# floatingtrees/video-VAE

Measured on AMD Instinct MI355X. Metric: video frames/sec (fwd+bwd) at Bx3x16x256x256, higher is better.
Workload: dtype bf16; 1 GPU; C3: full VideoVAE (enc 9 / dec 12 FactoredAttention + 3D-conv UNet) train step, B=4/GPU x 3x16x256x256, bf16 compute, fp32 params, recon+KL loss, clip+Adam; flavour=model, params=170631304, global_batch=4, frames_per_clip=16, parallelism=dp1, launch_mode=hipgraph(fwd+bwd) + eager all-reduce/clip/Adam

## Files before the change

### include/vvae_hip.h

```cpp
#ifndef VVAE_HIP_H
#define VVAE_HIP_H
#include <stddef.h>
#include <stdint.h>

#ifdef __cplusplus
extern "C" {
#endif

#define VVAE_DT_F32 0
#define VVAE_DT_BF16 1
#define VVAE_ERR_BAD_ARG 1001
#define VVAE_ERR_WORKSPACE 1002
#define VVAE_ERR_LIBRARY 1003

size_t vvae_conv3d_workspace_bytes(int N, int T, int H, int W, int Cin, int Cout, int kt, int kh, int kw, int dtype,
                                   int which );
int vvae_conv3d_fwd(const void* x, int ldx, const float* w, const float* bias, void* y, int ldy,
                    int N, int T, int H, int W, int Cin, int Cout, int kt, int kh, int kw, int dtype,
                    void* ws, size_t ws_bytes, void* stream);
int vvae_conv3d_dgrad(const void* dy, int lddy, const float* w, void* dx, int lddx,
                      int N, int T, int H, int W, int Cin, int Cout, int kt, int kh, int kw, int dtype,
                      void* ws, size_t ws_bytes, void* stream);
int vvae_conv3d_wgrad(const void* x, int ldx, const void* dy, int lddy, float* dw, float* dbias,
                      int N, int T, int H, int W, int Cin, int Cout, int kt, int kh, int kw, int dtype,
// ... 205 lines not shown
                          const float* sin_table, float* part, int A, int S, int heads, int D, float eps, int dtype, void* stream);

int vvae_layernorm_supported(int C, int dtype);
int vvae_layernorm_bwd_blocks(long rows, int C, int dtype);
int vvae_delay_us(int us, void* stream);
int vvae_layernorm_fwd_config(int fwd_cap);
int vvae_gn_config(int stream_blocks);
int vvae_layernorm_config(int bwd_cap);
int vvae_layernorm_fwd_mode(int late_stage);
int vvae_layernorm_fwd(const void* x, void* y, const float* gamma, const float* beta, float* mean, float* rstd,
                       const void* addend, void* xsum, long rows, int C, int inner, long outer_pitch, long inner_pitch, float eps,
                       int dtype, void* stream);
int vvae_layernorm_bwd(const void* x, const void* dy, const float* gamma, const float* mean, const float* rstd, const void* dres,
                       void* dx, float* part, long rows, int C, int inner, long outer_pitch, long inner_pitch, int dtype,
                       void* stream);

size_t vvae_loss_part_floats(int B, long M);
int vvae_reparam_kl_fwd(const void* mean, const void* logvar, const float* eps, const float* mask, float* z, float* kl,
                        float* part, int B, int T, long per, int dtype, void* stream);
int vvae_reparam_kl_bwd(const void* mean, const void* logvar, const float* eps, const float* mask, const float* dz,
                        const float* gkl, void* dmean, void* dlogvar, int B, int T, long per, int dtype, void* stream);

int vvae_masked_mse_mae_fwd(const void* video, const void* recon, const float* mask, float* mse, float* mae,
                            float* part, int B, int T, long P, int video_div, int dtype, void* stream);
int vvae_masked_mse_mae_bwd(const void* video, const void* recon, const float* mask, const float* gmse, const float* gmae,
                            void* drecon, int B, int T, long P, int video_div, int dtype, void* stream);

int vvae_gemm_tn_supported(int M, int N, int K, int lda, int ldb);
size_t vvae_gemm_tn_ws_bytes(int M, int N, int K);
int vvae_gemm_tn_bf16(const void* A, int lda, const void* B, int ldb, float* C, float* db, int M, int N, int K,
                      void* ws, size_t ws_bytes, void* stream);
int vvae_gemm_tn_grouped_bf16(const void* const* A, const int* lda, const void* const* B, const int* ldb, float* const* C,
                              float* const* db, const int* M, const int* N, int n, int K, void* stream);
int vvae_gemm_tn_use_big_tiles(int on);

int vvae_sqnorm_blocks(long n);
int vvae_sqnorm_partials(const float* g, long n, double* part, void* stream);
int vvae_adam_clip_step(float* p, const float* g, float* m, float* v, void* p_bf16, long n, const double* gnorm_part, int nparts,
                        double* gnorm_sq_out, float gscale, float max_norm, float lr, float b1, float b2, float eps, long count,
                        void* stream);
int vvae_cast_f32_to_bf16(const float* x, void* y, long n, void* stream);
int vvae_gemm_nt_supported(int M, int N, int K, int lda, int ldb, int ldc);
int vvae_gemm_nt_bf16(const void* A, int lda, const void* B, int ldb, void* C, int ldc, const float* bias, const void* res,
                      int ldr, void* C2, int ldc2, int epi, int M, int N, int K, void* stream);
int vvae_gemm_pp_supported(int M, int N, int K, int lda, int ldb, int ldc);
int vvae_gemm_pp_bf16(const void* A, int lda, const void* B, int ldb, void* C, int ldc, const float* bias, const void* res,
                      int ldr, void* C2, int ldc2, int epi, int M, int N, int K, void* stream);
int vvae_gemm_pp_ablate(int bits);
int vvae_gemm_pp_final_ring(int on);
int vvae_gemm_nt_stagger(int units);
int vvae_gemm_nt_persistent(int on);
int vvae_gemm_nt_prefetch(int dist);
int vvae_gemm_nt_prefetch_mask(int mask);

int vvae_sum_rows(const float* part, int rows, int cols, float* out, void* stream);
int vvae_fold_rows_grouped(const void* const* part, float* const* d0, float* const* d1, const int* rows, const int* cols,
                           const int* n0, int n, void* stream);
int vvae_copy_grouped(const float* const* src, float* const* dst, const long* count, int n, void* stream);

int vvae_selftest_xor_lane(const float* x, float* y, double* yd, int n, int o, void* stream);

#ifdef __cplusplus
}
#endif
#endif
```

### video_vae_amd/csrc/gemm_tn256.hip

```cpp
#include "common.hpp"

#ifndef TN_ABL
#define TN_ABL 0
#endif

namespace tn256 {

#ifdef TN_STAMPS
__device__ unsigned long long g_tn_stamps[256 * 4];
#endif

typedef __bf16 bf16x8 __attribute__((ext_vector_type(8)));
typedef short s16x4v __attribute__((ext_vector_type(4)));

constexpr int BM = 256, BN = 256, KS = 32, S = 4;
constexpr int ROW = 512;
constexpr int OPB = KS * ROW;
constexpr int STAGE = 2 * OPB;
constexpr int LDS_BYTES = S * STAGE;
constexpr int P = 4;
#ifndef TN_ALATE
#define TN_ALATE 3
#endif
constexpr int ALATE = TN_ALATE;

struct Dims { int M, N, K, lda, ldb, klen, tiles_m, tiles_n; };

template <int N> __device__ __forceinline__ void wait_vm()
{
    static_assert(N >= 0 && N < 64, "vmcnt is 6 bits");
    __builtin_amdgcn_s_waitcnt((N & 15) | ((N >> 4) << 14) | 0x0F70);
}

__device__ __forceinline__ void glds16(const void* g, unsigned char* lds_wave_base)
{
    __builtin_amdgcn_global_load_lds((const __attribute__((address_space(1))) void*)g,
                                     (__attribute__((address_space(3))) void*)lds_wave_base, 16, 0, 0);
}

__device__ __forceinline__ void tn256_tile(const bf16_t* __restrict__ A, const bf16_t* __restrict__ B, int lda, int ldb, int m0, int n0, int k_beg,
                                             int nk, float* __restrict__ out, int ld_out, float* __restrict__ out_db)
{
    extern __shared__ __attribute__((aligned(16))) unsigned char smem[];
    const int tid = threadIdx.x, lane = tid & 63, wave = tid >> 6;
    const int wm = wave >> 2, wn = wave & 3, grp = wave >> 2;

    const bf16_t* ga[2];
    const bf16_t* gb[2];
#pragma unroll
    for (int i = 0; i < 2; ++i) {
        const int row = 2 * (2 * wave + i) + (lane >> 5);
        const int chunk = (lane & 31) ^ ((row & 7) << 1);
        ga[i] = A + (long)(k_beg + row) * lda + m0 + chunk * 8;
        gb[i] = B + (long)(k_beg + row) * ldb + n0 + chunk * 8;
    }
    auto issue = [&](int t, int stage) {
        if ((TN_ABL & 1) && t >= S) return;
        unsigned char* sb = smem + stage * STAGE + (2 * wave) * 1024;
        const long ka = (long)t * KS * lda, kb = (long)t * KS * ldb;
        glds16(ga[0] + ka, sb);
        glds16(ga[1] + ka, sb + 1024);
        glds16(gb[0] + kb, sb + OPB);
        glds16(gb[1] + kb, sb + OPB + 1024);
    };
    auto wait_tiles = [&](int tiles_in_flight) {
        if (tiles_in_flight >= 2) wait_vm<2 * P>(); else if (tiles_in_flight == 1) wait_vm<P>(); else wait_vm<0>();
    };

    const int g4 = lane >> 4, q4 = (lane >> 2) & 3, p4 = lane & 3;
    const int r1 = 4 * g4 + q4, sw = (r1 & 7) << 1;
    int aoff[8], boff[4];
#pragma unroll
    for (int ib = 0; ib < 8; ++ib) aoff[ib] = r1 * ROW + ((((8 * wm + ib) * 2 + (p4 >> 1)) ^ sw) << 4) + (p4 & 1) * 8;
#pragma unroll
// ... 68 lines not shown
                    __builtin_amdgcn_sched_group_barrier(0x008, 2, 0);
                } else {
                    __builtin_amdgcn_sched_group_barrier(0x008, 4, 0);
                }
            }
        }
        if (do_bias && !(TN_ABL & 4)) {
#pragma unroll
            for (int jb = 0; jb < 4; ++jb) accb[jb] = __builtin_amdgcn_mfma_f32_16x16x32_bf16(ones, bfr[jb], accb[jb], 0, 0, 0);
        }
        asm volatile("s_waitcnt lgkmcnt(0)" ::: "memory");
        vvae_phase_barrier();
        st = st + 1 == S ? 0 : st + 1;
    }
    if (!grp) vvae_phase_barrier();
#ifdef TN_STAMPS
    if (tid == 0 && blockIdx.x < 256) { g_tn_stamps[blockIdx.x * 4 + 2] = __builtin_amdgcn_s_memtime(); g_tn_stamps[blockIdx.x * 4 + 3] = __builtin_amdgcn_s_memrealtime(); }
#endif

    const int nl = lane & 15;
#pragma unroll
    for (int ib = 0; ib < 8; ++ib)
#pragma unroll
        for (int jb = 0; jb < 4; ++jb)
#pragma unroll
            for (int j = 0; j < 4; ++j) {
                const int m = m0 + 128 * wm + 16 * ib + 4 * g4 + j;
                out[(long)m * ld_out + n0 + 64 * wn + 16 * jb + nl] = acc[ib][jb][j];
            }
    if (do_bias && g4 == 0) {
#pragma unroll
        for (int jb = 0; jb < 4; ++jb) out_db[n0 + 64 * wn + 16 * jb + nl] = accb[jb][0];
    }
}

__global__ __launch_bounds__(512, 1) void gemm_tn256_kernel(const bf16_t* __restrict__ A, const bf16_t* __restrict__ B, float* __restrict__ slab,
                                                            float* __restrict__ slab_db, Dims d)
{
    const int nwg = gridDim.x, q8 = nwg >> 3, r8 = nwg & 7, xcd = blockIdx.x & 7;
    const int L = (xcd < r8 ? xcd * (q8 + 1) : r8 * (q8 + 1) + (xcd - r8) * q8) + (blockIdx.x >> 3);
    const int tiles = d.tiles_m * d.tiles_n;
    const int sp = L / tiles, tile = L - sp * tiles;
    const int tm = tile / d.tiles_n, tn = tile - tm * d.tiles_n;
    const int k_beg = sp * d.klen;
    int k_end = k_beg + d.klen;
    if (k_end > d.K) k_end = d.K;
    tn256_tile(A, B, d.lda, d.ldb, tm * BM, tn * BN, k_beg, (k_end - k_beg) / KS, slab + (long)sp * d.M * d.N, d.N,
               (slab_db && tm == 0) ? slab_db + (long)sp * d.N : nullptr);
}

struct GroupProb { const bf16_t* A; const bf16_t* B; float* C; float* db; int M, N, lda, ldb, tiles_m, tiles_n, tile_start; };
constexpr int GROUP_MAX = 64;
struct GroupArgs { GroupProb p[GROUP_MAX]; int nprob, K; };

__global__ __launch_bounds__(512, 1) void gemm_tn256_grouped_kernel(GroupArgs g)
{
    const int nwg = gridDim.x, q8 = nwg >> 3, r8 = nwg & 7, xcd = blockIdx.x & 7;
    const int L = (xcd < r8 ? xcd * (q8 + 1) : r8 * (q8 + 1) + (xcd - r8) * q8) + (blockIdx.x >> 3);
    int pi = 0;
    for (int i = 1; i < g.nprob; ++i) pi = L >= g.p[i].tile_start ? i : pi;
    const GroupProb& P = g.p[pi];
    const int tile = L - P.tile_start;
    int tm, tn;
    if (P.tiles_m <= P.tiles_n) { tn = tile / P.tiles_m; tm = tile - tn * P.tiles_m; }
    else { tm = tile / P.tiles_n; tn = tile - tm * P.tiles_n; }
    tn256_tile(P.A, P.B, P.lda, P.ldb, tm * BM, tn * BN, 0, g.K / KS, P.C, P.N, (P.db && tm == 0) ? P.db : nullptr);
}

int pick_splits(int M, int N, int K)
{
    const int tiles = (M / BM) * (N / BN);
    int s = 256 / tiles;
    const int max_s = K / (8 * KS);
    if (s > max_s) s = max_s;
    if (s < 1) s = 1;
    return s;
}

bool supported(int M, int N, int K, int lda, int ldb)
{
    return M > 0 && N > 0 && K > 0 && M % BM == 0 && N % BN == 0 && K % KS == 0 && lda % 8 == 0 && ldb % 8 == 0 && lda >= M && ldb >= N;
}

int launch(const void* A, int lda, const void* B, int ldb, float* slab, float* slab_db, int M, int N, int K, int splits, int* used,
           hipStream_t s)
{
    int klen = (K + splits - 1) / splits;
    klen = (klen + KS - 1) / KS * KS;
    *used = (K + klen - 1) / klen;
    Dims d{M, N, K, lda, ldb, klen, M / BM, N / BN};
    static bool attr_done = false;
    if (!attr_done) {
        hipError_t e = hipFuncSetAttribute((const void*)gemm_tn256_kernel, hipFuncAttributeMaxDynamicSharedMemorySize, LDS_BYTES);
        if (e != hipSuccess) return (int)e;
        attr_done = true;
    }
    hipLaunchKernelGGL(gemm_tn256_kernel, dim3(d.tiles_m * d.tiles_n * *used), dim3(512), LDS_BYTES, s, (const bf16_t*)A, (const bf16_t*)B,
                       slab, slab_db, d);
    hipError_t e = hipGetLastError();
    return e == hipSuccess ? 0 : (int)e;
}

int launch_grouped(const GroupArgs& g, int total_tiles, hipStream_t s)
{
    static bool attr_done = false;
    if (!attr_done) {
        hipError_t e = hipFuncSetAttribute((const void*)gemm_tn256_grouped_kernel, hipFuncAttributeMaxDynamicSharedMemorySize, LDS_BYTES);
        if (e != hipSuccess) return (int)e;
        attr_done = true;
    }
    hipLaunchKernelGGL(gemm_tn256_grouped_kernel, dim3(total_tiles), dim3(512), LDS_BYTES, s, g);
    hipError_t e = hipGetLastError();
    return e == hipSuccess ? 0 : (int)e;
}

}

#ifdef TN_STAMPS
extern "C" int vvae_gemm_tn_stamps(unsigned long long* host_out)
{
    return (int)hipMemcpyFromSymbol(host_out, HIP_SYMBOL(tn256::g_tn_stamps), sizeof(unsigned long long) * 256 * 4, 0, hipMemcpyDeviceToHost);
}
#endif

extern "C" int vvae_gemm_tn_grouped_bf16(const void* const* A, const int* lda, const void* const* B, const int* ldb, float* const* C,
                                         float* const* db, const int* M, const int* N, int n, int K, void* stream)
{
    if (!A || !lda || !B || !ldb || !C || !db || !M || !N || n <= 0 || n > tn256::GROUP_MAX || K <= 0 || K % tn256::KS) return VVAE_ERR_BAD_ARG;
    tn256::GroupArgs g;
    g.nprob = n; g.K = K;
    int tiles = 0;
    for (int i = 0; i < n; ++i) {
        if (!A[i] || !B[i] || !C[i] || !tn256::supported(M[i], N[i], K, lda[i], ldb[i]) || ((uintptr_t)A[i] % 16) || ((uintptr_t)B[i] % 16) ||
            ((uintptr_t)C[i] % 16)) return VVAE_ERR_BAD_ARG;
        g.p[i] = tn256::GroupProb{(const bf16_t*)A[i], (const bf16_t*)B[i], C[i], db[i], M[i], N[i], lda[i], ldb[i], M[i] / tn256::BM,
                                  N[i] / tn256::BN, tiles};
        tiles += (M[i] / tn256::BM) * (N[i] / tn256::BN);
    }
    return tn256::launch_grouped(g, tiles, (hipStream_t)stream);
}
```

### video_vae_amd/csrc/loss_optim.hip

```cpp
#include "common.hpp"

namespace {

__device__ __forceinline__ float block_sum(float v, float* red) {
    v = wave_sum(v);
    const int lane = threadIdx.x & 63, wave = threadIdx.x >> 6;
    if (lane == 0) red[wave] = v;
    __syncthreads();
    float t = 0.f;
    if (threadIdx.x == 0) for (int i = 0; i < (int)(blockDim.x >> 6); ++i) t += red[i];
    __syncthreads();
    return t;
}

__device__ __forceinline__ float seq_len(const float* __restrict__ mrow, int T) {
    float s = 0.f;
    for (int t = 0; t < T; ++t) s += mrow[t];
    return fmaxf(s, 1.0f);
}

template <typename T_>
__global__ __launch_bounds__(256) void reparam_kl_fwd_kernel(const T_* __restrict__ mean, const T_* __restrict__ logvar,
                                                             const float* __restrict__ eps, const float* __restrict__ mask,
                                                             float* __restrict__ z, float* __restrict__ kl_part, int T, long per,
// ... 280 lines not shown
__global__ __launch_bounds__(256) void adam_clip_kernel(float* __restrict__ p, const float* __restrict__ g, float* __restrict__ m,
                                                        float* __restrict__ v, bf16_t* __restrict__ p_bf16, long n,
                                                        const double* __restrict__ gnorm_part, int nparts,
                                                        double* __restrict__ gnorm_sq_out, float gscale, float max_norm, float lr,
                                                        float b1, float b2, float eps, float c1, float c2)
{
    float clip = gscale;
    if (gnorm_part) {
        __shared__ double dred[256];
        double a = 0.0;
        for (int i = threadIdx.x; i < nparts; i += 256) a += gnorm_part[i];
        dred[threadIdx.x] = a;
        __syncthreads();
        for (int st = 128; st > 0; st >>= 1) {
            if ((int)threadIdx.x < st) dred[threadIdx.x] += dred[threadIdx.x + st];
            __syncthreads();
        }
        const double tot = dred[0];
        if (gnorm_sq_out && blockIdx.x == 0 && threadIdx.x == 0) *gnorm_sq_out = tot;
        const float gn = gscale * (float)sqrt(tot);
        if (gn >= max_norm) clip = gscale * max_norm / gn;
    }
    for (long i = (long)blockIdx.x * 256 + threadIdx.x; i < n; i += (long)gridDim.x * 256) {
        const float gi = g[i] * clip;
        const float mi = b1 * m[i] + (1.f - b1) * gi;
        const float vi = b2 * v[i] + (1.f - b2) * gi * gi;
        m[i] = mi; v[i] = vi;
        const float pi = p[i] - lr * (mi / c1) / (sqrtf(vi / c2) + eps);
        p[i] = pi;
        if (p_bf16) p_bf16[i] = f2bf(pi);
    }
}

__global__ __launch_bounds__(256) void cast_f32_bf16_kernel(const float* __restrict__ x, bf16_t* __restrict__ y, long n)
{
    for (long i = (long)blockIdx.x * 256 + threadIdx.x; i < n; i += (long)gridDim.x * 256) y[i] = f2bf(x[i]);
}

inline int pick_epb(long M, int B) {
    long want = 2048 / (B > 0 ? B : 1); if (want < 1) want = 1;
    long epb = (M + want - 1) / want;
    epb = ((epb + 2047) / 2048) * 2048;
    return (int)epb;
}

}

extern "C" size_t vvae_loss_part_floats(int B, long M)
{
    if (B <= 0 || M <= 0) return 0;
    return (size_t)2 * B * ceil_div(M, (long)pick_epb(M, B));
}

extern "C" int vvae_reparam_kl_fwd(const void* mean, const void* logvar, const float* eps, const float* mask, float* z, float* kl,
                                   float* part, int B, int T, long per, int dtype, void* stream)
{
    if (!mean || !logvar || (!z && !kl) || (z && !eps) || (kl && !part) || B <= 0 || T <= 0 || per <= 0) return VVAE_ERR_BAD_ARG;
    hipStream_t s = (hipStream_t)stream;
    const long M = (long)T * per;
    const int epb = pick_epb(M, B);
    dim3 grid(ceil_div(M, epb), B);
    float* klp = kl ? part : nullptr;
    if (dtype == VVAE_DT_F32)
        hipLaunchKernelGGL((reparam_kl_fwd_kernel<float>), grid, dim3(256), 0, s, (const float*)mean, (const float*)logvar, eps, mask, z, klp, T, per, epb);
    else if (dtype == VVAE_DT_BF16)
        hipLaunchKernelGGL((reparam_kl_fwd_kernel<bf16_t>), grid, dim3(256), 0, s, (const bf16_t*)mean, (const bf16_t*)logvar, eps, mask, z, klp, T, per, epb);
// ... 85 lines not shown
    } else return VVAE_ERR_BAD_ARG;
    VVAE_LAUNCH_CHECK();
    return 0;
}

extern "C" int vvae_sqnorm_blocks(long n)
{
    if (n <= 0) return 0;
    long blocks = n / 1024 + 1; if (blocks > SQN_MAX_BLOCKS) blocks = SQN_MAX_BLOCKS;
    return (int)blocks;
}

extern "C" int vvae_sqnorm_partials(const float* g, long n, double* part, void* stream)
{
    if (!g || !part || n <= 0 || ((uintptr_t)g % 16) != 0) return VVAE_ERR_BAD_ARG;
    hipLaunchKernelGGL(sqnorm_kernel, dim3((unsigned)vvae_sqnorm_blocks(n)), dim3(256), 0, (hipStream_t)stream, g, n, part);
    VVAE_LAUNCH_CHECK();
    return 0;
}

extern "C" int vvae_adam_clip_step(float* p, const float* g, float* m, float* v, void* p_bf16, long n, const double* gnorm_part,
                                   int nparts, double* gnorm_sq_out, float gscale, float max_norm, float lr, float b1, float b2,
                                   float eps, long count, void* stream)
{
    if (!p || !g || !m || !v || n <= 0 || count < 1 || (gnorm_part && (nparts <= 0 || nparts > SQN_MAX_BLOCKS))) return VVAE_ERR_BAD_ARG;
    const float c1 = 1.f - powf(b1, (float)count), c2 = 1.f - powf(b2, (float)count);
    long blocks = n / 1024 + 1; if (blocks > 4096) blocks = 4096;
    hipLaunchKernelGGL(adam_clip_kernel, dim3((unsigned)blocks), dim3(256), 0, (hipStream_t)stream, p, g, m, v, (bf16_t*)p_bf16, n,
                       gnorm_part, nparts, gnorm_sq_out, gscale, max_norm, lr, b1, b2, eps, c1, c2);
    VVAE_LAUNCH_CHECK();
    return 0;
}

extern "C" int vvae_cast_f32_to_bf16(const float* x, void* y, long n, void* stream)
{
    if (!x || !y || n <= 0) return VVAE_ERR_BAD_ARG;
    long blocks = n / 1024 + 1; if (blocks > 4096) blocks = 4096;
    hipLaunchKernelGGL(cast_f32_bf16_kernel, dim3((unsigned)blocks), dim3(256), 0, (hipStream_t)stream, x, (bf16_t*)y, n);
    VVAE_LAUNCH_CHECK();
    return 0;
}

namespace {
__global__ __launch_bounds__(256) void sum_rows_kernel(const float* __restrict__ part, int rows, int cols, float* __restrict__ out)
{
    __shared__ float4 red[32][8];
    const int cq = threadIdx.x & 7, rl = threadIdx.x >> 3;
    const int c = (blockIdx.x * 8 + cq) * 4;
    float4 s = make_float4(0.f, 0.f, 0.f, 0.f);
    if (c < cols) {
        for (int r0 = rl; r0 < rows; r0 += 32 * 16) {
            float4 v[16];
#pragma unroll
            for (int i = 0; i < 16; ++i) {
                const int r = r0 + 32 * i;
                v[i] = r < rows ? *reinterpret_cast<const float4*>(part + (long)r * cols + c) : make_float4(0.f, 0.f, 0.f, 0.f);
            }
#pragma unroll
            for (int i = 0; i < 16; ++i) { s.x += v[i].x; s.y += v[i].y; s.z += v[i].z; s.w += v[i].w; }
        }
    }
    red[rl][cq] = s;
    __syncthreads();
    for (int st = 16; st > 0; st >>= 1) {
        if (rl < st) {
            const float4 a = red[rl][cq], b = red[rl + st][cq];
// ... 251 lines not shown
```

### video_vae_amd/graph.py

```python
import ctypes
import gc

import torch

from . import loss as L
from . import ops


_NODE_TYPES = {0: "kernel", 1: "memcpy", 2: "memset", 3: "host", 4: "graph", 5: "empty", 6: "wait_event", 7: "event_record"}
_HIP = [None]


def graph_node_census(graph):
    raw = getattr(graph, "raw_cuda_graph", None)
    if raw is None:
        return None
    try:
        handle = raw()
        if _HIP[0] is None:
            _HIP[0] = ctypes.CDLL("libamdhip64.so")
        hip = _HIP[0]
        n = ctypes.c_size_t(0)
        if hip.hipGraphGetNodes(ctypes.c_void_p(handle), None, ctypes.byref(n)) != 0:
            return None
# ... 48 lines not shown
        self.graph = None
        self.debug_dot = debug_dot
        self._capture(warmup)

    @staticmethod
    def _unit(loss):
        return ops.unit_grad(loss) if (loss.dtype == torch.float32 and loss.dim() == 0) else None

    def _loss(self):
        emask = L.compact_mask(self.mask)
        if self.rl:
            return L.loss_fn(self.model, self.video, emask, self.mask, self.rngs, self.hparams, self.ploss, self.vgg_params)
        return L.loss_fn_plain(self.model, self.video, emask, self.mask, self.rngs, self.hparams)

    @staticmethod
    def _tensors(out):
        outs = out if isinstance(out, (tuple, list)) else (out,)
        return [o for o in outs if isinstance(o, torch.Tensor) and o.requires_grad]

    def _stage0(self):
        grabbed = {}
        hooks = [m.register_forward_hook(lambda mod, inp, out, j=j: grabbed.setdefault(j, []).append(out)) for j, m in enumerate(self.cut_modules)]
        try:
            loss, aux = self._loss()
        finally:
            for h in hooks:
                h.remove()
        self._cuts = []
        for j in range(len(self.cut_modules)):
            if len(grabbed.get(j, [])) != 1 or not self._tensors(grabbed[j][0]):
                raise RuntimeError("split capture expects every cut block of the encoder to run once and hand on differentiable tensors")
            self._cuts.append(self._tensors(grabbed[j][0]))
        opt = self.opt
        opt.external = set()
        opt.hooks_active = False
        params = [opt.params[i] for i in self.stage_idx[0]]
        with ops.deferred_wgrad(opt):
            grads = torch.autograd.grad(loss, params + self._cuts[0], grad_outputs=self._unit(loss), allow_unused=True)
        self._gcut = list(grads[len(params):])
        opt.land_subset(self.stage_idx[0], grads[:len(params)])
        return loss.detach(), {k: v.detach() for k, v in aux.items() if k != "reconstruction"}

    def _stage(self, st):
        opt = self.opt
        pairs = [(c, g) for c, g in zip(self._cuts[st - 1], self._gcut) if g is not None]
        params = [opt.params[i] for i in self.stage_idx[st]]
        nxt = self._cuts[st] if st < len(self._cuts) else []
        with ops.deferred_wgrad(opt):
            grads = torch.autograd.grad([c for c, _ in pairs], params + nxt, grad_outputs=[g for _, g in pairs], allow_unused=True)
        self._gcut = list(grads[len(params):])
        opt.land_subset(self.stage_idx[st], grads[:len(params)])
        if st == self.nstages - 1:
            opt.landed = [True] * len(opt.buckets)
            self._cuts = self._gcut = None

    def _prelaunch(self, st):
        opt = self.opt
        if opt.reducer is not None and opt.defer_reduce:
            if st == 0:
                opt.reducer.reset()
            for b, bs in enumerate(self.bucket_stage):
                if bs == st:
                    opt.reducer.launch(b)
                    opt.prelaunched.add(b)

    def _pass(self):
        if not self.split:
            return self._fwd_bwd()
        out = self._stage0()
        for st in range(1, self.nstages):
            self._prelaunch(st - 1)
            self._stage(st)
        return out

    def _fwd_bwd(self):
        loss, aux = self._loss()
        self.opt.external = set()
        self.opt.hooks_active = False
        with ops.deferred_wgrad(self.opt):
            grads = torch.autograd.grad(loss, self.opt.params, grad_outputs=self._unit(loss), allow_unused=True)
        self.opt.land_all(grads)
        return loss.detach(), {k: v.detach() for k, v in aux.items() if k != "reconstruction"}

    def _check_one_stream(self):
        from .optim import STREAM_TAG, accumulate_grad_node
        from ._lib import VvaeError
        if not self.video.is_cuda:
            return
        want = self.stream.cuda_stream
        with torch.cuda.stream(self.stream):
            for name, prm in zip(self.opt.names, self.opt.params):
                node = accumulate_grad_node(prm)
                have = node.metadata.get(STREAM_TAG) if node is not None else None
                if have is not None and have != want:
                    raise VvaeError(
                        f"GraphedTrainStep: parameter {name!r} has already taken part in an eager backward on stream {have:#x} and that pass's "
                        f"autograd graph is still alive, but the capture would run on stream {want:#x}.  One stream for the whole run: build the "
                        "model, run the eager steps and capture on the same non-default stream (pass it as stream=..., as train.py does), or drop "
                        "every tensor of the eager passes (loss, aux) before capturing.")

    def _refill(self):
        for name, (kind, buf) in self.noise.items():
            buf.normal_(generator=self.gen) if kind == "normal" else buf.uniform_(generator=self.gen)

    def _capture(self, warmup):
        opt = self.opt
        self.stream = self.capture_stream if self.capture_stream is not None else torch.cuda.Stream()
        self.stream.wait_stream(torch.cuda.current_stream())
        if getattr(self.model, "_kl", None) is not None:
            self.model._kl = None
# ... 22 lines not shown
            opt.zero_grad()
        torch.cuda.synchronize()
        gc.collect()
        try:
            g = torch.cuda.CUDAGraph(keep_graph=True)
        except TypeError:
            g = torch.cuda.CUDAGraph()
        if self.debug_dot:
            g.enable_debug_mode()
        mode = "thread_local" if opt.reducer is not None else "global"
        if self.split:
            with torch.cuda.graph(g, stream=self.stream, capture_error_mode=mode):
                self.loss, self.aux = self._stage0()
            for st in range(1, self.nstages):
                try:
                    gs = torch.cuda.CUDAGraph(keep_graph=True)
                except TypeError:
                    gs = torch.cuda.CUDAGraph()
                with torch.cuda.graph(gs, stream=self.stream, pool=g.pool(), capture_error_mode=mode):
                    self._stage(st)
                self.graphs.append(gs)
        else:
            with torch.cuda.graph(g, stream=self.stream, capture_error_mode=mode):
                self.loss, self.aux = self._fwd_bwd()
        if not all(opt.landed):
            raise RuntimeError("a gradient bucket did not land inside the captured backward (parameter without gradient)")
        self.census = [graph_node_census(x) for x in [g] + self.graphs]
        for c in self.census:
            if c and c.get("memset", 0):
                raise RuntimeError(f"the captured train step holds {c['memset']} hipGraph memset node(s) ({c}): on ROCm 7.2 a replayed memset node writes "
                                   "garbage, and whatever it was meant to zero (e.g. the semaphore of a multi-block framework reduction) misbehaves on "
                                   "replay.  Replace the op that issued hipMemsetAsync (DESIGN.md section 3, tools/memset_node_probe.py).")
        self.graph = g
        if self.debug_dot:
            g.debug_dump(self.debug_dot)
        opt.update()
        with torch.no_grad():
            opt.p.copy_(snap[0]); opt.m.copy_(snap[1]); opt.v.copy_(snap[2])
        opt.count = snap[3]
        opt.refresh_shadow()

    def __call__(self, video=None, mask=None, noise=None):
        if video is not None:
            self.video.copy_(video)
        if mask is not None:
            self.mask.copy_(mask)
        if noise is None:
            self._refill()
        else:
            if set(noise) != set(self.noise):
                raise KeyError(f"noise for {sorted(noise)} given, the captured step draws {sorted(self.noise)}")
            for name, t in noise.items():
                self.noise[name][1].copy_(t)
        self.graph.replay()
        for st, gs in enumerate(self.graphs, start=1):
            self._prelaunch(st - 1)
            gs.replay()
        self.opt.update()
        return self.loss, self.aux
```

### video_vae_amd/ops.py

```python
import ctypes
import os
import sys

import torch
import torch.nn.functional as F

from ._lib import lib, check, VvaeError

DT = {torch.float32: 0, torch.bfloat16: 1}

_NOTED = set()


def note_fallback(key, message):
    if key in _NOTED:
        return
    _NOTED.add(key)
    import os
    import sys
    if os.environ.get("RANK", "0") == "0":
        print(f"[video_vae_amd] fallback: {message}", file=sys.stderr, flush=True)


def _stream():
# ... 2038 lines not shown
        x2, dy2, kernel, bias = item
        self.claim(kernel)
        t = (x2.shape[1] // 256) * (dy2.shape[1] // 256)
        if self.items and (x2.shape[0] != self.k or len(self.items) == GROUP_MAX or self.tiles + t > GROUP_TILES):
            self.flush()
        self.items.append(item); self.tiles += t; self.k = x2.shape[0]

    def flush(self):
        items, tiles, k = self.items, self.tiles, self.k
        self.items, self.tiles = [], 0
        if items:
            flush_wgrad(items, self.opt, tiles, k)


def wgrad_deferrable(x2, dy2, kernel, bias):
    if WGRAD_QUEUE[0] is None or getattr(kernel, "gview", None) is None or (bias is not None and getattr(bias, "gview", None) is None):
        return False
    k, m = x2.shape
    n = dy2.shape[1]
    return (x2.is_cuda and x2.dtype == torch.bfloat16 and dy2.dtype == torch.bfloat16 and x2.stride(1) == 1 and dy2.stride(1) == 1
            and m % 256 == 0 and n % 256 == 0 and k % 32 == 0 and x2.stride(0) % 8 == 0 and dy2.stride(0) % 8 == 0
            and x2.data_ptr() % 16 == 0 and dy2.data_ptr() % 16 == 0)


def flush_wgrad(items, optimizer, tiles=None, k=None):
    if not items:
        return
    if tiles is None:
        tiles = sum((x2.shape[1] // 256) * (dy2.shape[1] // 256) for x2, dy2, _, _ in items)
        k = items[0][0].shape[0]
    if os.environ.get("VVAE_WGRAD_DEBUG"):
        print(f"[vvae] dense dW flush: {len(items)} products, {tiles} tiles of 256 x 256, K {k}: " + ("grouped" if tiles >= GROUP_MIN_TILES else "per product"), file=sys.stderr)
    if tiles >= GROUP_MIN_TILES:
        _gemm_tn_grouped(items, k)
    else:
        for x2, dy2, kernel, bias in items:
            gemm_tn(x2, dy2, bias is not None, kernel.gview, bias.gview if bias is not None else None)
    for _, _, kernel, bias in items:
        optimizer.mark_external(kernel)
        if bias is not None:
            optimizer.mark_external(bias)


def _gemm_tn_grouped(chunk, k):
    n = len(chunk)
    VP, IA = ctypes.c_void_p * n, ctypes.c_int * n
    a = VP(*[x2.data_ptr() for x2, _, _, _ in chunk])
    b = VP(*[dy2.data_ptr() for _, dy2, _, _ in chunk])
    c = VP(*[kn.gview.data_ptr() for _, _, kn, _ in chunk])
    db = VP(*[(bi.gview.data_ptr() if bi is not None else None) for _, _, _, bi in chunk])
    lda = IA(*[x2.stride(0) for x2, _, _, _ in chunk])
    ldb = IA(*[dy2.stride(0) for _, dy2, _, _ in chunk])
    ms = IA(*[x2.shape[1] for x2, _, _, _ in chunk])
    ns = IA(*[dy2.shape[1] for _, dy2, _, _ in chunk])
    flops = sum(2 * k * x2.shape[1] * dy2.shape[1] for x2, dy2, _, _ in chunk)
    nbytes = sum(k * (x2.shape[1] + dy2.shape[1]) * 2 + x2.shape[1] * dy2.shape[1] * 4 for x2, dy2, _, _ in chunk)
    check(_launch(f"gemm_tn_grouped x{n} K{k}", nbytes, flops, "gemm_tn256_grouped_kernel",
                  lambda: lib().vvae_gemm_tn_grouped_bf16(a, lda, b, ldb, c, db, ms, ns, n, k, _stream())), "vvae_gemm_tn_grouped_bf16")


def gemm_tn_supported(a, b):
    return (a.is_cuda and a.dtype == torch.bfloat16 and b.dtype == torch.bfloat16 and a.dim() == 2 and b.dim() == 2
            and a.stride(1) == 1 and b.stride(1) == 1
            and lib().vvae_gemm_tn_supported(a.shape[1], b.shape[1], a.shape[0], a.stride(0), b.stride(0)) == 1)


def gemm_tn(a, b, want_colsum=True, out=None, out_colsum=None):
    k, m = a.shape
    n = b.shape[1]
    c = out if out is not None else torch.empty((m, n), dtype=torch.float32, device=a.device)
    db = (out_colsum if out_colsum is not None else torch.empty((n,), dtype=torch.float32, device=a.device)) if want_colsum else None
    assert c.is_contiguous() and c.dtype == torch.float32 and c.shape == (m, n)
    wsb = lib().vvae_gemm_tn_ws_bytes(m, n, k)
    ws, wsb = _ws(wsb, a.device)
    kern = ("gemm_tn256_kernel" if m % 256 == 0 and n % 256 == 0 and k % 32 == 0 else "gemm_tn_bf16_kernel") + " + gemm_tn_reduce_kernel"
    check(_launch(f"gemm_tn {m}x{n} K{k}", (k * (m + n)) * 2 + m * n * 4, 2 * m * n * k, kern,
                  lambda: lib().vvae_gemm_tn_bf16(_p(a), a.stride(0), _p(b), b.stride(0), _p(c), _p(db), m, n, k, _p(ws), wsb, _stream())),
          "vvae_gemm_tn_bf16")
    return c, db
```

### video_vae_amd/optim.py

```python
import ctypes
import math

import torch

from ._lib import lib, check


def warmup_cosine_decay_schedule(init_value, peak_value, warmup_steps, decay_steps, end_value):
    def schedule(count):
        if count < warmup_steps:
            return init_value + (peak_value - init_value) * (count / warmup_steps)
        span = decay_steps - warmup_steps
        c = min(count - warmup_steps, span)
        cosine = 0.5 * (1.0 + math.cos(math.pi * c / span))
        alpha = end_value / peak_value
        return peak_value * ((1 - alpha) * cosine + alpha)
    return schedule


def reference_schedule(batch_size=2, learning_rate=2e-5, decay_steps=1_000_000):
    return warmup_cosine_decay_schedule(0.0, learning_rate, 20000 // math.sqrt(batch_size), decay_steps, learning_rate / 10)


def _copy_all(dsts, srcs):
    from . import ops
    fast = [(d, s) for d, s in zip(dsts, srcs) if ops.copy_grouped_ok(d, s)]
    rest = [(d, s) for d, s in zip(dsts, srcs) if not ops.copy_grouped_ok(d, s)]
    if fast:
        ops.copy_grouped([d for d, _ in fast], [s for _, s in fast])
    if rest:
        torch._foreach_copy_([d for d, _ in rest], [s for _, s in rest])


STREAM_TAG = "vvae_accumulate_stream"


def accumulate_grad_node(param):
    with torch.enable_grad():
        fn = param.expand_as(param).grad_fn
    nxt = fn.next_functions if fn is not None else ()
    return nxt[0][0] if nxt and nxt[0][0] is not None else None


class Optimizer:

    def __init__(self, model, schedule, max_norm=1.0, b1=0.9, b2=0.999, eps=1e-8, bf16_shadow=True,
                 bucket_bytes=64 << 20):
        self.model = model
        self.schedule = schedule if callable(schedule) else (lambda count, lr=schedule: lr)
        self.max_norm, self.b1, self.b2, self.eps = max_norm, b1, b2, eps
        self.count = 0
        named = [(n, p) for n, p in model.named_parameters() if p.requires_grad]
        self.names = [n for n, _ in named][::-1]
        self.params = [p for _, p in named][::-1]
        dev = self.params[0].device
        for p in self.params:
            if p.dtype != torch.float32:
                raise ValueError("Optimizer expects fp32 parameters (param_dtype=float32)")
        self.offsets, off = [], 0
        for p in self.params:
            self.offsets.append(off)
            off += (p.numel() + 3) // 4 * 4
        self.numel = off
        self.p = torch.zeros(off, dtype=torch.float32, device=dev)
        self.g = torch.zeros(off, dtype=torch.float32, device=dev)
        self.m = torch.zeros(off, dtype=torch.float32, device=dev)
        self.v = torch.zeros(off, dtype=torch.float32, device=dev)
        self.gnorm_sq = torch.zeros(1, dtype=torch.float64, device=dev)
        self.gnorm_part = torch.zeros(max(1, lib().vvae_sqnorm_blocks(off)) if dev.type == "cuda" else 1, dtype=torch.float64, device=dev)
        self.shadow = torch.zeros(off, dtype=torch.bfloat16, device=dev) if bf16_shadow else None
        self.gviews = []
        for p, o in zip(self.params, self.offsets):
            n = p.numel()
            self.p[o:o + n].copy_(p.data.reshape(-1))
            p.data = self.p[o:o + n].view(p.shape)
            p.grad = None
            self.gviews.append(self.g[o:o + n].view(p.shape))
            p.gview = self.gviews[-1]
            if self.shadow is not None:
                p.bf16 = self.shadow[o:o + n].view(p.shape)
        if self.shadow is not None:
            self.shadow.copy_(self.p)
        self.tpairs = []
        if self.shadow is not None and dev.type == "cuda":
            want = [p for p in self.params if getattr(p, "want_t", False) and p.dim() == 2 and p.shape[0] % 64 == 0 and p.shape[1] % 64 == 0
                    and p.bf16.data_ptr() % 16 == 0]
            if want:
                tbuf = torch.zeros(sum(p.numel() for p in want), dtype=torch.bfloat16, device=dev)
                o = 0
                for p in want:
                    p.bf16_t = tbuf[o:o + p.numel()].view(p.shape[1], p.shape[0])
                    self.tpairs.append((p.bf16, p.bf16_t))
                    o += p.numel()
                self._refresh_transposed()
        cap = max(1, bucket_bytes // 4)
        ends = [o + (p.numel() + 3) // 4 * 4 for o, p in zip(self.offsets, self.params)]
        self.buckets, self.param_bucket, self.bucket_params = [], [], []
        start, members = 0, []
        for i, e in enumerate(ends):
            self.param_bucket.append(len(self.buckets))
            members.append(i)
            if e - start >= cap or i == len(ends) - 1:
# ... 63 lines not shown
            if gr is None:
                if i not in self.clean:
                    gv.zero_()
                    self.clean.add(i)
            else:
                self.clean.discard(i)
                dsts.append(gv)
                srcs.append(gr)
        if dsts:
            _copy_all(dsts, srcs)
        self.landed = [True] * len(self.buckets)
        if self.reducer is not None and not self.defer_reduce:
            for b in range(len(self.buckets)):
                self.reducer.launch(b)

    @torch.no_grad()
    def land_subset(self, indices, grads):
        dsts, srcs = [], []
        for i, gr in zip(indices, grads):
            if i in self.external:
                self.clean.discard(i)
                continue
            if gr is None:
                if i not in self.clean:
                    self.gviews[i].zero_()
                    self.clean.add(i)
            else:
                self.clean.discard(i)
                dsts.append(self.gviews[i])
                srcs.append(gr)
        if dsts:
            _copy_all(dsts, srcs)

    def mark_external(self, param):
        i = self.index[id(param)]
        self.external.add(i)
        if self.hooks_active:
            b = self.param_bucket[i]
            self.arrived[b] += 1
            if self.arrived[b] == len(self.bucket_params[b]) and not self.landed[b]:
                self._land(b)

    def zero_grad(self):
        self.external = set()
        for p in self.params:
            p.grad = None
        self.arrived = [0] * len(self.buckets)
        self.landed = [False] * len(self.buckets)
        if self.reducer is not None:
            self.reducer.reset()

    def set_grads(self, grads):
        self.zero_grad()
        by_name = dict(zip(self.names, range(len(self.names))))
        for n, gr in grads.items():
            i = by_name[n]
            self.params[i].grad = gr.to(self.g.device)
        for b in range(len(self.buckets)):
            self._land(b)

    @torch.no_grad()
    def update(self):
        for b in range(len(self.buckets)):
            if not self.landed[b]:
                self._land(b)
        gscale = 1.0
        if self.reducer is not None:
            if self.defer_reduce:
                if not self.prelaunched:
                    self.reducer.reset()
                for b in range(len(self.buckets)):
                    if b not in self.prelaunched:
                        self.reducer.launch(b)
                self.prelaunched = set()
            self.reducer.finish()
            gscale = 1.0 / self.reducer.world_size
        if not self.p.is_cuda:
            raise RuntimeError("Optimizer.update runs the fused HIP clip+Adam kernel and needs GPU parameters")
        s = ctypes.c_void_p(torch.cuda.current_stream().cuda_stream)
        lr = float(self.schedule(self.count))
        self.count += 1
        vp = lambda t: ctypes.c_void_p(t.data_ptr())
        check(lib().vvae_sqnorm_partials(vp(self.g), self.numel, vp(self.gnorm_part), s), "vvae_sqnorm_partials")
        check(lib().vvae_adam_clip_step(vp(self.p), vp(self.g), vp(self.m), vp(self.v),
                                        vp(self.shadow) if self.shadow is not None else None, self.numel, vp(self.gnorm_part),
                                        self.gnorm_part.numel(), vp(self.gnorm_sq), gscale, self.max_norm, lr, self.b1, self.b2,
                                        self.eps, self.count, s),
              "vvae_adam_clip_step")
        if self.tpairs:
            self._refresh_transposed()
        self.last_lr = lr
        return lr

    def _refresh_transposed(self):
        s = ctypes.c_void_p(torch.cuda.current_stream().cuda_stream)
        for i0 in range(0, len(self.tpairs), 64):
            e = self.tpairs[i0:i0 + 64]
            n = len(e)
            VP, IA = ctypes.c_void_p * n, ctypes.c_int * n
            check(lib().vvae_transpose_grouped_bf16(VP(*[a.data_ptr() for a, _ in e]), VP(*[b.data_ptr() for _, b in e]),
                                                    IA(*[a.shape[0] for a, _ in e]), IA(*[a.shape[1] for a, _ in e]), n, s),
                  "vvae_transpose_grouped_bf16")

    def refresh_shadow(self):
        if self.shadow is not None:
            self.shadow.copy_(self.p)
            if self.tpairs:
                self._refresh_transposed()

    def grad_norm(self):
        scale = 1.0 / self.reducer.world_size if self.reducer is not None else 1.0
        return float(self.gnorm_sq.item()) ** 0.5 * scale

    def state_dict(self):
        out = {"count": self.count}
        for n, p, o in zip(self.names, self.params, self.offsets):
            k = p.numel()
            out[f"mu.{n}"] = self.m[o:o + k].view(p.shape).detach().cpu().clone()
            out[f"nu.{n}"] = self.v[o:o + k].view(p.shape).detach().cpu().clone()
# ... 10 lines not shown
```

Measured before the change: 1999 frames/s.

## Fuse gradient squared-norm partials into grouped dW GEMM epilogue

The grouped weight-gradient GEMM now computes per-tile sums of squares of its output (and bias grads) and writes them to an optimizer-owned partials buffer. The optimizer then runs a reduced sqnorm kernel that reads only the gradient ranges not covered by these writers and folds in the GEMM partials. This avoids re-reading most of the 170M-element gradient buffer before clip+Adam. It adds epilogue work and a block sync to each GEMM tile, plus claim/state bookkeeping that must be saved and restored around graph replay.

```diff
diff --git a/include/vvae_hip.h b/include/vvae_hip.h
--- a/include/vvae_hip.h
+++ b/include/vvae_hip.h
@@ -261,6 +261,8 @@
                       void* ws, size_t ws_bytes, void* stream);
 int vvae_gemm_tn_grouped_bf16(const void* const* A, const int* lda, const void* const* B, const int* ldb, float* const* C,
                               float* const* db, const int* M, const int* N, int n, int K, void* stream);
+int vvae_gemm_tn_grouped_sq_bf16(const void* const* A, const int* lda, const void* const* B, const int* ldb, float* const* C,
+                                 float* const* db, const int* M, const int* N, int n, int K, double* sq_part, void* stream);
 int vvae_gemm_tn_use_big_tiles(int on);
 
 int vvae_sqnorm_blocks(long n);
@@ -268,6 +270,7 @@
 int vvae_adam_clip_step(float* p, const float* g, float* m, float* v, void* p_bf16, long n, const double* gnorm_part, int nparts,
                         double* gnorm_sq_out, float gscale, float max_norm, float lr, float b1, float b2, float eps, long count,
                         void* stream);
+int vvae_sqnorm_items(const float* g, const long* items, int nitems, const double* wpart, int nw, double* part, void* stream);
 int vvae_cast_f32_to_bf16(const float* x, void* y, long n, void* stream);
 int vvae_gemm_nt_supported(int M, int N, int K, int lda, int ldb, int ldc);
 int vvae_gemm_nt_bf16(const void* A, int lda, const void* B, int ldb, void* C, int ldc, const float* bias, const void* res,
diff --git a/video_vae_amd/csrc/gemm_tn256.hip b/video_vae_amd/csrc/gemm_tn256.hip
--- a/video_vae_amd/csrc/gemm_tn256.hip
+++ b/video_vae_amd/csrc/gemm_tn256.hip
@@ -39,7 +39,7 @@
 }
 
 __device__ __forceinline__ void tn256_tile(const bf16_t* __restrict__ A, const bf16_t* __restrict__ B, int lda, int ldb, int m0, int n0, int k_beg,
-                                             int nk, float* __restrict__ out, int ld_out, float* __restrict__ out_db)
+                                             int nk, float* __restrict__ out, int ld_out, float* __restrict__ out_db, double* __restrict__ sq_out = nullptr)
 {
     extern __shared__ __attribute__((aligned(16))) unsigned char smem[];
     const int tid = threadIdx.x, lane = tid & 63, wave = tid >> 6;
@@ -174,6 +174,29 @@
 #pragma unroll
         for (int jb = 0; jb < 4; ++jb) out_db[n0 + 64 * wn + 16 * jb + nl] = accb[jb][0];
     }
+    if (sq_out) {
+        float sq = 0.f;
+#pragma unroll
+        for (int ib = 0; ib < 8; ++ib)
+#pragma unroll
+            for (int jb = 0; jb < 4; ++jb)
+#pragma unroll
+                for (int j = 0; j < 4; ++j) sq += acc[ib][jb][j] * acc[ib][jb][j];
+        if (do_bias && g4 == 0) {
+#pragma unroll
+            for (int jb = 0; jb < 4; ++jb) sq += accb[jb][0] * accb[jb][0];
+        }
+        sq = wave_sum(sq);
+        float* red = reinterpret_cast<float*>(smem);
+        if (lane == 0) red[wave] = sq;
+        __syncthreads();
+        if (tid == 0) {
+            double t = 0.0;
+#pragma unroll
+            for (int w = 0; w < 8; ++w) t += (double)red[w];
+            *sq_out = t;
+        }
+    }
 }
 
 __global__ __launch_bounds__(512, 1) void gemm_tn256_kernel(const bf16_t* __restrict__ A, const bf16_t* __restrict__ B, float* __restrict__ slab,
@@ -193,7 +216,7 @@
 
 struct GroupProb { const bf16_t* A; const bf16_t* B; float* C; float* db; int M, N, lda, ldb, tiles_m, tiles_n, tile_start; };
 constexpr int GROUP_MAX = 64;
-struct GroupArgs { GroupProb p[GROUP_MAX]; int nprob, K; };
+struct GroupArgs { GroupProb p[GROUP_MAX]; int nprob, K; double* sq; };
 
 __global__ __launch_bounds__(512, 1) void gemm_tn256_grouped_kernel(GroupArgs g)
 {
@@ -206,7 +229,8 @@
     int tm, tn;
     if (P.tiles_m <= P.tiles_n) { tn = tile / P.tiles_m; tm = tile - tn * P.tiles_m; }
     else { tm = tile / P.tiles_n; tn = tile - tm * P.tiles_n; }
-    tn256_tile(P.A, P.B, P.lda, P.ldb, tm * BM, tn * BN, 0, g.K / KS, P.C, P.N, (P.db && tm == 0) ? P.db : nullptr);
+    tn256_tile(P.A, P.B, P.lda, P.ldb, tm * BM, tn * BN, 0, g.K / KS, P.C, P.N, (P.db && tm == 0) ? P.db : nullptr,
+               g.sq ? g.sq + blockIdx.x : nullptr);
 }
 
 int pick_splits(int M, int N, int K)
@@ -265,12 +289,12 @@
 }
 #endif
 
-extern "C" int vvae_gemm_tn_grouped_bf16(const void* const* A, const int* lda, const void* const* B, const int* ldb, float* const* C,
-                                         float* const* db, const int* M, const int* N, int n, int K, void* stream)
+extern "C" int vvae_gemm_tn_grouped_sq_bf16(const void* const* A, const int* lda, const void* const* B, const int* ldb, float* const* C,
+                                            float* const* db, const int* M, const int* N, int n, int K, double* sq_part, void* stream)
 {
     if (!A || !lda || !B || !ldb || !C || !db || !M || !N || n <= 0 || n > tn256::GROUP_MAX || K <= 0 || K % tn256::KS) return VVAE_ERR_BAD_ARG;
     tn256::GroupArgs g;
-    g.nprob = n; g.K = K;
+    g.nprob = n; g.K = K; g.sq = sq_part;
     int tiles = 0;
     for (int i = 0; i < n; ++i) {
         if (!A[i] || !B[i] || !C[i] || !tn256::supported(M[i], N[i], K, lda[i], ldb[i]) || ((uintptr_t)A[i] % 16) || ((uintptr_t)B[i] % 16) ||
@@ -281,3 +305,9 @@
     }
     return tn256::launch_grouped(g, tiles, (hipStream_t)stream);
 }
+
+extern "C" int vvae_gemm_tn_grouped_bf16(const void* const* A, const int* lda, const void* const* B, const int* ldb, float* const* C,
+                                         float* const* db, const int* M, const int* N, int n, int K, void* stream)
+{
+    return vvae_gemm_tn_grouped_sq_bf16(A, lda, B, ldb, C, db, M, N, n, K, nullptr, stream);
+}
diff --git a/video_vae_amd/csrc/loss_optim.hip b/video_vae_amd/csrc/loss_optim.hip
--- a/video_vae_amd/csrc/loss_optim.hip
+++ b/video_vae_amd/csrc/loss_optim.hip
@@ -336,6 +336,30 @@
     }
 }
 
+__global__ __launch_bounds__(256) void sqnorm_items_kernel(const float* __restrict__ g, const long* __restrict__ items,
+                                                           const double* __restrict__ wpart, int nw, double* __restrict__ part)
+{
+    __shared__ float red[4];
+    __shared__ double dred[256];
+    const long n4 = items[2 * blockIdx.x + 1];
+    const float4* g4 = reinterpret_cast<const float4*>(g) + items[2 * blockIdx.x];
+    float acc = 0.f;
+    for (long i = threadIdx.x; i < n4; i += 256) {
+        const float4 t = g4[i];
+        acc += t.x * t.x + t.y * t.y + t.z * t.z + t.w * t.w;
+    }
+    const float t = block_sum(acc, red);
+    double a = 0.0;
+    for (long i = (long)blockIdx.x * 256 + threadIdx.x; i < nw; i += (long)gridDim.x * 256) a += wpart[i];
+    dred[threadIdx.x] = a;
+    __syncthreads();
+    for (int st = 128; st > 0; st >>= 1) {
+        if ((int)threadIdx.x < st) dred[threadIdx.x] += dred[threadIdx.x + st];
+        __syncthreads();
+    }
+    if (threadIdx.x == 0) part[blockIdx.x] = (double)t + dred[0];
+}
+
 __global__ __launch_bounds__(256) void cast_f32_bf16_kernel(const float* __restrict__ x, bf16_t* __restrict__ y, long n)
 {
     for (long i = (long)blockIdx.x * 256 + threadIdx.x; i < n; i += (long)gridDim.x * 256) y[i] = f2bf(x[i]);
@@ -487,6 +511,14 @@
     return 0;
 }
 
+extern "C" int vvae_sqnorm_items(const float* g, const long* items, int nitems, const double* wpart, int nw, double* part, void* stream)
+{
+    if (!g || !items || !part || nitems <= 0 || nitems > SQN_MAX_BLOCKS || nw < 0 || (nw > 0 && !wpart) || ((uintptr_t)g % 16) != 0) return VVAE_ERR_BAD_ARG;
+    hipLaunchKernelGGL(sqnorm_items_kernel, dim3((unsigned)nitems), dim3(256), 0, (hipStream_t)stream, g, items, wpart, nw, part);
+    VVAE_LAUNCH_CHECK();
+    return 0;
+}
+
 extern "C" int vvae_cast_f32_to_bf16(const float* x, void* y, long n, void* stream)
 {
     if (!x || !y || n <= 0) return VVAE_ERR_BAD_ARG;
diff --git a/video_vae_amd/graph.py b/video_vae_amd/graph.py
--- a/video_vae_amd/graph.py
+++ b/video_vae_amd/graph.py
@@ -104,7 +104,7 @@
                 raise RuntimeError("split capture expects every cut block of the encoder to run once and hand on differentiable tensors")
             self._cuts.append(self._tensors(grabbed[j][0]))
         opt = self.opt
-        opt.external = set()
+        opt.reset_external()
         opt.hooks_active = False
         params = [opt.params[i] for i in self.stage_idx[0]]
         with ops.deferred_wgrad(opt):
@@ -147,7 +147,7 @@
 
     def _fwd_bwd(self):
         loss, aux = self._loss()
-        self.opt.external = set()
+        self.opt.reset_external()
         self.opt.hooks_active = False
         with ops.deferred_wgrad(self.opt):
             grads = torch.autograd.grad(loss, self.opt.params, grad_outputs=self._unit(loss), allow_unused=True)
@@ -236,6 +236,7 @@
                                    "garbage, and whatever it was meant to zero (e.g. the semaphore of a multi-block framework reduction) misbehaves on "
                                    "replay.  Replace the op that issued hipMemsetAsync (DESIGN.md section 3, tools/memset_node_probe.py).")
         self.graph = g
+        self._sq_state = opt.sq_state()
         if self.debug_dot:
             g.debug_dump(self.debug_dot)
         opt.update()
@@ -260,5 +261,6 @@
         for st, gs in enumerate(self.graphs, start=1):
             self._prelaunch(st - 1)
             gs.replay()
+        self.opt.set_sq_state(self._sq_state)
         self.opt.update()
         return self.loss, self.aux
diff --git a/video_vae_amd/ops.py b/video_vae_amd/ops.py
--- a/video_vae_amd/ops.py
+++ b/video_vae_amd/ops.py
@@ -2094,7 +2094,7 @@
     if os.environ.get("VVAE_WGRAD_DEBUG"):
         print(f"[vvae] dense dW flush: {len(items)} products, {tiles} tiles of 256 x 256, K {k}: " + ("grouped" if tiles >= GROUP_MIN_TILES else "per product"), file=sys.stderr)
     if tiles >= GROUP_MIN_TILES:
-        _gemm_tn_grouped(items, k)
+        _gemm_tn_grouped(items, k, optimizer)
     else:
         for x2, dy2, kernel, bias in items:
             gemm_tn(x2, dy2, bias is not None, kernel.gview, bias.gview if bias is not None else None)
@@ -2104,8 +2104,13 @@
             optimizer.mark_external(bias)
 
 
-def _gemm_tn_grouped(chunk, k):
+def _gemm_tn_grouped(chunk, k, optimizer=None):
     n = len(chunk)
+    sq = None
+    claim = getattr(optimizer, "claim_sq_partials", None)
+    if claim is not None:
+        tiles = sum((x2.shape[1] // 256) * (dy2.shape[1] // 256) for x2, dy2, _, _ in chunk)
+        sq = claim([q for _, _, kn, bi in chunk for q in ((kn,) if bi is None else (kn, bi))], tiles)
     VP, IA = ctypes.c_void_p * n, ctypes.c_int * n
     a = VP(*[x2.data_ptr() for x2, _, _, _ in chunk])
     b = VP(*[dy2.data_ptr() for _, dy2, _, _ in chunk])
@@ -2118,7 +2123,8 @@
     flops = sum(2 * k * x2.shape[1] * dy2.shape[1] for x2, dy2, _, _ in chunk)
     nbytes = sum(k * (x2.shape[1] + dy2.shape[1]) * 2 + x2.shape[1] * dy2.shape[1] * 4 for x2, dy2, _, _ in chunk)
     check(_launch(f"gemm_tn_grouped x{n} K{k}", nbytes, flops, "gemm_tn256_grouped_kernel",
-                  lambda: lib().vvae_gemm_tn_grouped_bf16(a, lda, b, ldb, c, db, ms, ns, n, k, _stream())), "vvae_gemm_tn_grouped_bf16")
+                  lambda: lib().vvae_gemm_tn_grouped_sq_bf16(a, lda, b, ldb, c, db, ms, ns, n, k, ctypes.c_void_p(sq), _stream())),
+          "vvae_gemm_tn_grouped_sq_bf16")
 
 
 def gemm_tn_supported(a, b):
diff --git a/video_vae_amd/optim.py b/video_vae_amd/optim.py
--- a/video_vae_amd/optim.py
+++ b/video_vae_amd/optim.py
@@ -1,5 +1,6 @@
 import ctypes
 import math
+import os
 
 import torch
 
@@ -32,6 +33,30 @@
         torch._foreach_copy_([d for d, _ in rest], [s for _, s in rest])
 
 
+SQN_MAX_ITEMS = 1024
+
+
+def leftover_items(offsets, sizes, total, covered, max_items=SQN_MAX_ITEMS):
+    ranges, pos = [], 0
+    for i in sorted(covered, key=lambda j: offsets[j]):
+        o, e = offsets[i], offsets[i] + (sizes[i] + 3) // 4 * 4
+        if o > pos:
+            ranges.append((pos, o))
+        pos = max(pos, e)
+    if pos < total:
+        ranges.append((pos, total))
+    if len(ranges) >= max_items:
+        return None
+    left4 = sum(e - o for o, e in ranges) // 4
+    chunk = max(4096, -(-left4 // max(1, max_items - len(ranges))))
+    items = []
+    for o, e in ranges:
+        for b in range(o // 4, e // 4, chunk):
+            items.append((b, min(chunk, e // 4 - b)))
+    return items or [(0, 0)]
+
+
+WRITER_NORM = os.environ.get("VVAE_WRITER_NORM", "1") != "0"
 STREAM_TAG = "vvae_accumulate_stream"
 
 
@@ -67,7 +92,13 @@
         self.m = torch.zeros(off, dtype=torch.float32, device=dev)
         self.v = torch.zeros(off, dtype=torch.float32, device=dev)
         self.gnorm_sq = torch.zeros(1, dtype=torch.float64, device=dev)
-        self.gnorm_part = torch.zeros(max(1, lib().vvae_sqnorm_blocks(off)) if dev.type == "cuda" else 1, dtype=torch.float64, device=dev)
+        self.gnorm_blocks = max(1, lib().vvae_sqnorm_blocks(off)) if dev.type == "cuda" else 1
+        self.gnorm_part = torch.zeros(max(self.gnorm_blocks, SQN_MAX_ITEMS), dtype=torch.float64, device=dev)
+        self.writer_norm = WRITER_NORM
+        tiles = sum((p.shape[0] // 256) * (p.shape[1] // 256) for p in self.params if p.dim() == 2 and p.shape[0] % 256 == 0 and p.shape[1] % 256 == 0)
+        self.sq_part = torch.zeros(tiles, dtype=torch.float64, device=dev) if tiles and dev.type == "cuda" else None
+        self.sq_claims, self.sq_used = {}, 0
+        self._items = {}
         self.shadow = torch.zeros(off, dtype=torch.bfloat16, device=dev) if bf16_shadow else None
         self.gviews = []
         for p, o in zip(self.params, self.offsets):
@@ -197,6 +228,34 @@
         if dsts:
             _copy_all(dsts, srcs)
 
+    def reset_external(self):
+        self.external = set()
+        self.sq_claims, self.sq_used = {}, 0
+        self.writer_norm = WRITER_NORM
+
+    def claim_sq_partials(self, params, tiles):
+        if not self.writer_norm or self.reducer is not None or self.sq_part is None or self.sq_used + tiles > self.sq_part.numel():
+            return None
+        idx = [self.index.get(id(p)) for p in params]
+        if any(i is None or i in self.sq_claims for i in idx):
+            return None
+        base, self.sq_used = self.sq_used, self.sq_used + tiles
+        self.sq_claims.update((i, base) for i in idx)
+        return self.sq_part.data_ptr() + 8 * base
+
+    def sq_state(self):
+        return dict(self.sq_claims), self.sq_used, set(self.external), self.writer_norm
+
+    def set_sq_state(self, state):
+        self.sq_claims, self.sq_used, self.external, self.writer_norm = dict(state[0]), state[1], set(state[2]), state[3]
+
+    def _leftover_table(self):
+        key = tuple(sorted(self.sq_claims))
+        if key not in self._items:
+            items = leftover_items(self.offsets, [p.numel() for p in self.params], self.numel, key)
+            self._items[key] = (torch.tensor(items, dtype=torch.int64).to(self.g.device), len(items)) if items is not None else None
+        return self._items[key]
+
     def mark_external(self, param):
         i = self.index[id(param)]
         self.external.add(i)
@@ -207,7 +266,7 @@
                 self._land(b)
 
     def zero_grad(self):
-        self.external = set()
+        self.reset_external()
         for p in self.params:
             p.grad = None
         self.arrived = [0] * len(self.buckets)
@@ -246,10 +305,20 @@
         lr = float(self.schedule(self.count))
         self.count += 1
         vp = lambda t: ctypes.c_void_p(t.data_ptr())
-        check(lib().vvae_sqnorm_partials(vp(self.g), self.numel, vp(self.gnorm_part), s), "vvae_sqnorm_partials")
+        left = None
+        if self.writer_norm and self.reducer is None and self.sq_claims and all(i in self.external for i in self.sq_claims):
+            left = self._leftover_table()
+        if left is not None:
+            nparts = left[1]
+            check(lib().vvae_sqnorm_items(vp(self.g), vp(left[0]), nparts, vp(self.sq_part), self.sq_used, vp(self.gnorm_part), s),
+                  "vvae_sqnorm_items")
+        else:
+            nparts = self.gnorm_blocks
+            check(lib().vvae_sqnorm_partials(vp(self.g), self.numel, vp(self.gnorm_part), s), "vvae_sqnorm_partials")
+        self.norm_path = "writers" if left is not None else "full"
         check(lib().vvae_adam_clip_step(vp(self.p), vp(self.g), vp(self.m), vp(self.v),
                                         vp(self.shadow) if self.shadow is not None else None, self.numel, vp(self.gnorm_part),
-                                        self.gnorm_part.numel(), vp(self.gnorm_sq), gscale, self.max_norm, lr, self.b1, self.b2,
+                                        nparts, vp(self.gnorm_sq), gscale, self.max_norm, lr, self.b1, self.b2,
                                         self.eps, self.count, s),
               "vvae_adam_clip_step")
         if self.tpairs:
```

Result: no change. 2005 frames/s, median of 6 (+0.3%).
